# DavidRother/cooking_zoo

Measured on AMD Instinct MI355X. Metric: env-steps/sec at N parallel envs (1/2/4/8 GPU) + achieved HBM GB/s, higher is better.
Workload: dtype u8/u32 state, f64 obs+reward

## Files before the change

### cooking_zoo_amd/csrc/cz_api.hip

```cpp
#include <hip/hip_runtime.h>
#include <dlfcn.h>
#include <stdarg.h>
#include <stdio.h>
#include <stdlib.h>
#include <string.h>

#include <atomic>
#include <string>
#include <vector>

#include "../../include/cookingzoo.h"
#include "cz_launch.h"
#include "cz_generate.h"

using namespace cz;

constexpr int STAT_CHAINS = 256, STAT_COLS = 13;
__global__ __launch_bounds__(64) void k_stats_chains(const uint32_t *__restrict__ su, const double *__restrict__ sf,
                                                     const uint32_t *__restrict__ state, int RW, int N,
                                                     unsigned long long *__restrict__ part ) {
    const int chain = (int)blockIdx.x * 4 + ((int)threadIdx.x >> 4), col = (int)threadIdx.x & 15;
    const int widx = col == 0 ? (int)SU_STEPS : col == 1 ? (int)SU_EPISODES : col == 2 ? (int)SU_LENSUM : col == 3 ? (int)SU_TRUNC
                   : col == 4 ? (int)SU_TERM : col < 9 ? (int)SU_COMPLETED0 + col - 5 : 0;
    const int fidx = (col >= 9 && col < STAT_COLS) ? (int)SF_SUM0 + col - 9 : (int)SF_SUM0;
// ... 264 lines not shown
        double *obs = nullptr, *rew = nullptr; uint8_t *term = nullptr, *trunc = nullptr; hipStream_t stream = nullptr; uint64_t version = 0;
        bool operator==(const RingKey &o) const {
            return ring == o.ring && stride == o.stride && period == o.period && obs == o.obs && rew == o.rew && term == o.term &&
                   trunc == o.trunc && stream == o.stream && version == o.version;
        }
    } ring_key;
    struct RunGraph { int32_t slot, len; hipGraphExec_t ge; uint64_t used; };
    std::vector<RunGraph> ring_graphs;
    uint64_t ring_clock = 0;
    int64_t n_graph_kernels = 0, n_direct_kernels = 0;
    uint64_t tables_version = 0;
    hipEvent_t ev0 = nullptr, ev1 = nullptr;
    bool ktime = false;
    std::vector<hipEvent_t> kev;
    size_t kev_used = 0;
    double ktime_ms = 0.0;
    int64_t klaunches = 0;
    void *rccl = nullptr;
    void *comm = nullptr;
    int n_ranks = 1, rank = 0;
    int wt_override = -1;
    bool lean_enabled = true;
    bool lean_cfg_enabled = true;
    int last_step_variant = -1;
    int last_step_lean = -1;
    int last_step_mode = -1;
    bool huge = false;
    int instance = 0;
    unsigned long long *tl_base = nullptr;
    int32_t tl_cap = 0;
    int64_t tl_count = 0;
    bool graphs_enabled = true;
    bool ring_fused = false;
    int64_t n_ring_fused_steps = 0;
    int32_t graph_min_run = 48;
    int32_t ring_prefix = 0;
    size_t zero_copy_bytes = (size_t)256 << 10;
    cz_stats *d_gather = nullptr;
    std::string err;
};

static thread_local std::string g_err;
static int ready(cz_handle h);
static int set_device(cz_handle h);
static int begin_ranged_call(cz_handle h, int64_t b, int64_t c);
static void mark_ranks(cz_handle h, int32_t first, int32_t count, int ok);
static int flush_updates(cz_handle h, bool force);
// ... 101 lines not shown
    int ndev = 0;
    if (hipGetDeviceCount(&ndev) != hipSuccess || ndev == 0)
        return fail(nullptr, "cz_create: no HIP device available (this library has no CPU fallback)");
    if (cfg->device_id < 0 || cfg->device_id >= ndev) return fail(nullptr, "cz_create: device_id %d out of range", cfg->device_id);
    cz_handle h = new cz_handle_s();
    h->cfg = *cfg;
#define CREATE_CHK(call)                                                                          \
    do {                                                                                          \
        hipError_t _e = (call);                                                                   \
        if (_e != hipSuccess) {                                                                   \
            fail(nullptr, "cz_create: %s failed: %s", #call, hipGetErrorString(_e));             \
            cz_destroy(h);                                                                        \
            return 1;                                                                             \
        }                                                                                         \
    } while (0)
    CREATE_CHK(hipSetDevice(cfg->device_id));
    CREATE_CHK(hipStreamCreateWithFlags(&h->own_stream, hipStreamNonBlocking));
    h->stream = h->own_stream;
    CREATE_CHK(hipEventCreate(&h->ev0));
    CREATE_CHK(hipEventCreate(&h->ev1));
    Params &P = h->P;
    memset(&P, 0, sizeof P);
    P.N = cfg->num_envs; P.A = cfg->num_agents; P.W = cfg->width; P.H = cfg->height; P.D = cfg->max_dyn; P.F = cfg->feat_len;
    const int CW = (C + 3) / 4;
    P.dyn0_off = CELL_WORD0 + CW;
    P.dyn1_off = P.dyn0_off + P.D;
    P.RW = (P.dyn1_off + P.D + 15) / 16 * 16;
    P.scheme = cfg->action_scheme; P.max_steps = cfg->max_steps; P.end_all = cfg->end_condition_all ? 1 : 0;
    P.R = cfg->num_recipes; P.auto_reset = cfg->auto_reset ? 1 : 0; P.env_id_base = cfg->env_id_base;
    P.recipe_reward = cfg->recipe_reward; P.recipe_penalty = cfg->recipe_penalty; P.node_reward = cfg->recipe_node_reward;
    P.time_penalty_step = cfg->max_time_penalty / (double)cfg->max_steps;
    P.T = 1;
    if (const char *s = getenv("CZ_WT")) h->wt_override = atoi(s);
    if (const char *s = getenv("CZ_LEAN")) h->lean_enabled = atoi(s) != 0;
    if (const char *s = getenv("CZ_LEAN_CFG")) h->lean_cfg_enabled = atoi(s) != 0;
    if (const char *s = getenv("CZ_GRAPHS")) h->graphs_enabled = atoi(s) != 0;
    if (const char *s = getenv("CZ_GRAPH_MIN_RUN")) h->graph_min_run = atoi(s) < 4 ? 4 : (atoi(s) > 256 ? 256 : atoi(s));
    if (const char *s = getenv("CZ_RING_PREFIX")) h->ring_prefix = atoi(s) < 0 ? 0 : (atoi(s) > 16 ? 16 : atoi(s));
    if (const char *s = getenv("CZ_ZERO_COPY_BYTES")) h->zero_copy_bytes = (size_t)atoll(s);
#ifdef CZ_SMALL_ONLY
    if (!(P.D <= 64 && C <= 64)) { fail(nullptr, "cz_create: this diagnostic library holds the small kernel instance only"); cz_destroy(h); return 1; }
    h->kl = launchers_small();
#else
    h->instance = (P.D <= 64 && C <= 64) ? 0 : (P.D <= 128 && C <= 256) ? 1 : 2;
    h->kl = h->instance == 0 ? launchers_small() : h->instance == 1 ? launchers_large() : launchers_huge();
#endif
    h->huge = P.D > 128 || C > 256;
    {
        double x = 0.0;
        x += (double)0 * P.node_reward;
        x += 0.0 * P.recipe_reward;
        x += 0.0 * P.recipe_penalty;
        x += P.time_penalty_step;
        P.reward_idle = x;
    }
    const size_t N = (size_t)P.N;
    const size_t state_bytes = N * P.RW * 4;
    CREATE_CHK(hipMalloc(&h->d_state, state_bytes));
// ... 607 lines not shown
};
enum ObsForm { OBS_F64, OBS_CODES, OBS_F32 };

static const char *resolve_step(cz_handle h, const StepCall &c, Params &P, ObsForm &form) {
    uint8_t *const codes = c.fused || c.codes ? c.codes : h->codes;
    float *const obs32 = c.fused || c.obs32 ? c.obs32 : h->obs32;
    if (obs32) {
        if (codes) return "a float32 output (cz_set_f32_output / cz_step_device_f32) and a compact output (cz_set_compact_output / "
                          "cz_step_device_compact) are both set: switch one of them off";
        if (c.obs) return "float32 observation rows are switched on (cz_set_f32_output): pass d_obs = NULL, or switch them off "
                          "with cz_set_f32_output(h, NULL) to get float64 rows";
    }
    form = obs32 ? OBS_F32 : codes ? OBS_CODES : OBS_F64;
    P = h->P;
    P.actions = c.actions; P.obs = c.obs; P.rewards = c.rewards; P.term = c.term; P.trunc = c.trunc; P.marks_out = c.marks;
    P.T = c.T; P.seed = c.seed; P.step0 = c.step0;
    if (obs32) P.obs32 = obs32; else P.codes = codes;
    return nullptr;
}

static hipError_t choose_step(cz_handle h, const Params &P, bool fused, ObsForm form, StepChoice &c) {
    c.lean = false;
    c.cfg = -1;
    if (fused && form == OBS_F32) c.mode = P.actions ? ROLLOUT_ACTIONS_F32 : ROLLOUT_F32;
    else if (fused) c.mode = P.actions ? ROLLOUT_ACTIONS : form != OBS_CODES ? ROLLOUT : P.obs ? ROLLOUT_CODES : ROLLOUT_CODES_ONLY;
    else c.mode = form == OBS_F32 ? STEP_F32 : form == OBS_CODES ? STEP_CODES : STEP;
    if (c.mode == STEP)
        c.lean = h->lean_enabled && h->kl.has_lean && P.obs && !P.marks_out && !P.wide && !(P.auto_reset & 2) && P.F <= 128 * OBS_PAIRS && P.wt == 1;
    if (c.lean && h->lean_cfg_enabled) c.cfg = lean_cfg_of(P);
    return !fused && !P.actions ? hipErrorInvalidValue : hipSuccess;
}

static int launch_step(cz_handle h, const StepCall &call) {
    if ((h->P.auto_reset & 2) && h->spawn_layouts != h->n_layouts)
        return fail(h, "despawn / respawn is on, but the layout pool was reloaded since cz_set_spawn (now %d layouts): call cz_set_spawn "
                       "again (it maps every layout to the level whose spawn areas it uses)", h->n_layouts);
    const hipStream_t stream = h->stream;
    const bool fused = call.fused;
    Params P;
    ObsForm form;
    if (const char *refused = resolve_step(h, call, P, form)) return fail(h, "%s", refused);
    const bool f32 = form == OBS_F32;
    const size_t obs_bytes = (size_t)P.N * P.A * P.F * (f32 ? 4 : 8);
    if (!fused) P.wt = obs_bytes > ((size_t)224 << 20) ? 2 : P.N <= 10240 ? 1 : 0;
    else P.wt = (obs_bytes > ((size_t)224 << 20) && (size_t)P.F * (f32 ? 4 : 8) >= 4096) ? 2 : 0;
    if (h->wt_override >= 0) P.wt = h->wt_override;
    if (!fused) {
        if (!P.rewards) P.rewards = (double *)h->d_dump;
        if (!P.term) P.term = (uint8_t *)h->d_dump;
        if (!P.trunc) P.trunc = (uint8_t *)h->d_dump;
    }
#ifdef CZ_TIMELINE
    P.timeline = (h->tl_base && h->tl_cap > 0) ? h->tl_base + (size_t)(h->tl_count++ % h->tl_cap) * (size_t)P.N * 2 : nullptr;
#endif
    hipEvent_t e0 = nullptr, e1 = nullptr;
    if (h->ktime && caller_capturing(h)) return fail(h, "kernel timing (cz_kernel_time_reset) cannot run inside a stream capture of the caller");
    if (h->ktime) {
        while (h->kev.size() < h->kev_used + 2) {
            hipEvent_t e;
            HIPCHK(h, hipEventCreate(&e));
            h->kev.push_back(e);
        }
        e0 = h->kev[h->kev_used]; e1 = h->kev[h->kev_used + 1];
        h->kev_used += 2;
        HIPCHK(h, hipEventRecord(e0, stream));
    }
    StepChoice choice;
    const hipError_t chosen = choose_step(h, P, fused, form, choice);
    h->last_step_lean = choice.lean ? 1 : 0;
    h->last_step_mode = choice.mode;
    h->last_step_variant = !choice.lean ? -1 : choice.cfg < 0 ? 0 : (0x100 | P.R | (P.end_all << 4) | (P.walk_touches << 5));
    HIPCHK(h, chosen);
    HIPCHK(h, h->kl.step(P, stream, choice));
    if (h->ktime) HIPCHK(h, hipEventRecord(e1, stream));
    return 0;
}
extern "C" int cz_reset(cz_handle h, int64_t b, int64_t c, const int32_t *layout_ids, const uint8_t *recipe_ids,
                        const uint32_t *pool_words, double *obs) {
    if (ready(h) || check_range(h, b, c)) return 1;
    if (c == 0) return 0;
    if (!layout_ids || !recipe_ids) return fail(h, "cz_reset: null argument");
    HIPCHK(h, hipSetDevice(h->cfg.device_id));
    std::vector<uint32_t> pools((size_t)c, 0u);
    for (int64_t i = 0; i < c; ++i) {
        if (layout_ids[i] < 0 || layout_ids[i] >= h->n_layouts) return fail(h, "cz_reset: layout id %d out of range", layout_ids[i]);
        for (int r = 0; r < h->P.R; ++r)
            if (recipe_ids[i * 4 + r] >= h->n_recipes) return fail(h, "cz_reset: recipe id %d out of range", recipe_ids[i * 4 + r]);
        if (pool_words) {
            uint32_t base = pool_words[i] & 0xFFFFu, count = pool_words[i] >> 16;
            if (count && (int)(base + count) > h->n_layouts) return fail(h, "cz_reset: layout pool slice [%u,%u) out of range", base, base + count);
            pools[(size_t)i] = pool_words[i];
        }
    }
    int32_t *const d_lay = h->d_reset_words;
// ... 356 lines not shown
extern "C" int64_t cz_partner_bad_recipes(cz_handle h) {
    if (!h || !h->d_partner) return h ? 0 : -1;
    return read_counter<unsigned long long>(h, partner_counter(h), "cz_partner_bad_recipes");
}
extern "C" int32_t cz_num_actions(cz_handle h) { return h ? (h->P.scheme == 3 ? 5 : 8) : -1; }
extern "C" int cz_action_effects_device(cz_handle h, int64_t b, int64_t c, uint32_t agents, uint32_t ignore, uint8_t *d_mask, uint8_t *d_effects) {
    if (begin_ranged_call(h, b, c)) return 1;
    if (agents == 0 || agents >> h->P.A) return fail(h, "cz_action_effects_device: agents is 0x%x, not a non-empty set of the %d agents", agents, h->P.A);
    if (ignore & ~FX_ALL) return fail(h, "cz_action_effects_device: unknown ignore bits 0x%x", ignore & ~FX_ALL);
    if (!d_mask && !d_effects) return fail(h, "cz_action_effects_device: both output pointers are null");
    if (c == 0) return 0;
    if (set_device(h)) return 1;
    HIPCHK(h, h->kl.action_effects(h->P, h->stream, (int)c, EffectsArgs{b, agents, ignore, d_mask, d_effects}));
    return 0;
}
extern "C" int cz_obs_table_f32(cz_handle h, float *table) {
    if (!h || !table) return fail(h, "cz_obs_table_f32: null argument");
    for (int i = 0; i < LUT_SIZE; ++i) table[i] = (float)h->obs_table[i];
    return 0;
}
extern "C" int32_t cz_diag_last_step_lean(cz_handle h) { return h ? h->last_step_lean : -1; }
extern "C" int32_t cz_diag_last_step_mode(cz_handle h) { return h ? h->last_step_mode : -1; }
extern "C" int32_t cz_diag_last_step_variant(cz_handle h) { return h ? h->last_step_variant : -1; }
extern "C" int32_t cz_diag_instance(cz_handle h) { return h ? h->instance : -1; }
extern "C" int cz_diag_read_layout_pool(cz_handle h, int32_t first, int32_t count, uint32_t *records, uint32_t *desc) {
    if (ready(h)) return 1;
    if (!h->d_lay_init || !h->d_lay_desc) return fail(h, "cz_diag_read_layout_pool: no layout pool loaded");
    if (first < 0 || count < 0 || (int64_t)first + count > h->n_layouts)
        return fail(h, "cz_diag_read_layout_pool: slots [%d, %d) outside the resident pool of %d layouts", first, first + count, h->n_layouts);
    if (count == 0) return 0;
    if (set_device(h)) return 1;
    HIPCHK(h, hipStreamSynchronize(h->stream));
    if (records)
        HIPCHK(h, hipMemcpy(records, h->d_lay_init + (size_t)first * h->P.RW, (size_t)count * h->P.RW * 4, hipMemcpyDeviceToHost));
    if (desc)
        HIPCHK(h, hipMemcpy(desc, h->d_lay_desc + (size_t)first * h->P.F, (size_t)count * h->P.F * 4, hipMemcpyDeviceToHost));
    return 0;
}
extern "C" int cz_obs_table(cz_handle h, double *table) {
    if (!h || !table) return fail(h, "cz_obs_table: null argument");
    memcpy(table, h->obs_table, sizeof h->obs_table);
    return 0;
}
extern "C" const void *cz_obs_table_device(cz_handle h) { return h ? (const void *)h->d_lut : nullptr; }

static bool ring_fusable(cz_handle h, const StepCall &c, int32_t K, int64_t stride);
// ... 593 lines not shown
```

### cooking_zoo_amd/csrc/cz_device.h

```cpp
#pragma once
#include <hip/hip_runtime.h>
#include <stdint.h>
#include <type_traits>

namespace cz {

constexpr int MAX_AGENTS = 4;
constexpr int MAX_NODES = 8;
constexpr int WIDE_NODES = 16;
constexpr int HDR_WORDS = 8;
constexpr int AGENT_WORD0 = HDR_WORDS;
constexpr int RET_WORD0 = HDR_WORDS + MAX_AGENTS;
constexpr int CELL_WORD0 = RET_WORD0 + 2 * MAX_AGENTS;

enum : uint32_t { FLOOR = 0, COUNTER, DELIVERSQUARE, SWITCH, BLOCK, CUTBOARD, BLENDER };
enum : uint32_t { PLATE = 0, ONION, TOMATO, LETTUCE, CARROT, CUCUMBER, BANANA, APPLE, WATERMELON, BREAD };
enum : uint32_t { CELL_TYPE = 7, CELL_READY = 8, CELL_TOGGLE = 16, CELL_ACTIVE = 32, CELL_WALK = 64 };
enum : uint32_t { D_ALIVE = 1u << 24, D_CHOPPED = 2u << 24, D_MASHED = 4u << 24, D_FREE = 8u << 24, D_DONE = 6u << 24 };
enum : uint32_t { COND_NONE = 0, COND_CHOPPED, COND_MASHED, COND_NOT_CHOPPED, COND_NOT_MASHED };
enum : uint32_t { W_T = 0, W_MARKS, W_LAYOUT, W_STATUS, W_EPISODE, W_RECIPES, W_POOL, W_MARKS_HI };
enum : uint32_t { ST_DONE = 1, ST_TERM = 2, ST_TRUNC = 4 };
constexpr int LUT_Y0 = 63, LUT_ZERO = 126, LUT_ONE = 127;
constexpr int LUT_NDONE0 = 128, LUT_CH0 = 132, LUT_MA0 = 136, LUT_CF0 = 140, LUT_OR0 = 144;
enum : uint32_t { SU_EPISODES = 0, SU_STEPS, SU_LENSUM, SU_TRUNC, SU_TERM, SU_COMPLETED0, SU_LAST_LENGTH = 9, SU_LAST_EPISODE, SU_LAST_FLAGS,
// ... 69 lines not shown
static_assert(LEADING_SCALAR_BYTES + sizeof(LeanParams) <= 4 * 64, "the lean argument block: four 64-byte lines with the leading scalars");
#endif
static_assert(LEADING_SCALAR_BYTES + offsetof(LeanParams, obs) + sizeof(double *) == 2 * 64, "the common path's fields end the second line");
struct LeanView : LeanParams {
    uint32_t *state;
    const int32_t *actions;
    const double *lut;
    int32_t N, RW, W, H, D, dyn0_off, dyn1_off;
    static constexpr int32_t wide = 0, wt = 1, T = 1;
    static constexpr uint32_t step0 = 0u;
    static constexpr uint64_t seed = 0u;
    static constexpr uint8_t *codes = nullptr;
    int32_t R, end_all, walk_touches;
    LeanView() = default;
    __host__ __device__ explicit LeanView(const LeanParams &b)
        : LeanParams(b), R((int32_t)(b.settings & 0xFFu)), end_all((int32_t)((b.settings >> 8) & 1u)), walk_touches((int32_t)((b.settings >> 16) & 1u)) {}
};
template <int R_, int END_ALL, int WALK_TOUCHES>
struct LeanViewFixed : LeanView {
    static_assert(R_ >= 1 && R_ <= 4 && (END_ALL | 1) == 1 && (WALK_TOUCHES | 1) == 1, "no such handle");
    static constexpr int32_t R = R_, end_all = END_ALL, walk_touches = WALK_TOUCHES;
    using LeanView::LeanView;
};
template <class PB> using block_of = std::conditional_t<std::is_base_of<LeanParams, PB>::value, LeanParams, Params>;

#ifndef CZ_PRIO
#define CZ_PRIO 1
#endif
#if CZ_PRIO
#define CZ_SETPRIO(p) __builtin_amdgcn_s_setprio(p)
#else
#define CZ_SETPRIO(p) do { } while (0)
#endif
__device__ __forceinline__ uint32_t rfl(uint32_t v) { return __builtin_amdgcn_readfirstlane(v); }
__device__ __forceinline__ uint32_t rdl(uint32_t v, int l) { return __builtin_amdgcn_readlane(v, l); }
__device__ __forceinline__ uint64_t ballot(bool p) { return __builtin_amdgcn_ballot_w64(p); }
__device__ __forceinline__ bool lanes(uint64_t m) { return __builtin_amdgcn_inverse_ballot_w64(m); }
extern "C" __device__ uint32_t __cz_writelane(uint32_t, uint32_t, uint32_t) __asm("llvm.amdgcn.writelane.i32");
__device__ __forceinline__ uint32_t wrl(uint32_t value, int lane, uint32_t into) { return __cz_writelane(value, (uint32_t)lane, into); }

__host__ __device__ inline uint32_t action_hash(uint64_t seed, int64_t env_global, int agent, uint32_t step, uint32_t n) {
    uint32_t x = (uint32_t)seed ^ ((uint32_t)(seed >> 32) * 0x9E3779B1u);
    x ^= (uint32_t)env_global * 0x85EBCA6Bu + (uint32_t)((uint64_t)env_global >> 32) * 0x27D4EB2Fu;
    x ^= ((uint32_t)agent + 1u) * 0xC2B2AE35u;
    x ^= (step + 1u) * 0x165667B1u;
    x ^= x >> 16; x *= 0x7FEB352Du; x ^= x >> 15; x *= 0x846CA68Bu; x ^= x >> 16;
// ... 859 lines not shown
```

### cooking_zoo_amd/csrc/cz_kernels.h

```cpp
#pragma once
#include "cz_device.h"
#include <type_traits>

namespace cz {

#ifdef CZ_PROFILE
#define CZ_STAMP(i)                                                                                    \
    do {                                                                                               \
        unsigned long long _t;                                                                         \
        __builtin_amdgcn_sched_barrier(0);                                                             \
        asm volatile("s_memrealtime %0\n\ts_waitcnt lgkmcnt(0)" : "=s"(_t)::"memory");                 \
        __builtin_amdgcn_sched_barrier(0);                                                             \
        if (lane == 0 && P.stamps) P.stamps[(size_t)env * 16 + (i)] = _t;                               \
    } while (0)
#elif defined(CZ_MARKERS)
#define CZ_STAMP(i) asm volatile("; CZ_MARK " #i)
#else
#define CZ_STAMP(i) do { } while (0)
#endif

typedef const __attribute__((address_space(4))) Params *KParams;
struct StepArgsMirror { uint32_t *a; const int32_t *b; const double *c; int32_t i[8]; Params p; };
struct LeanArgsMirror { uint32_t *a; const int32_t *b; const double *c; int32_t i[8]; LeanParams p; };
static_assert(offsetof(LeanArgsMirror, p) == LEADING_SCALAR_BYTES && offsetof(StepArgsMirror, p) == LEADING_SCALAR_BYTES, "leading scalars");
// ... 22 lines not shown
};
template <int MODE, bool LEAN = false>
struct StepTraits {
    static_assert(MODE >= STEP && MODE <= ROLLOUT_ACTIONS_F32 && (!LEAN || MODE == STEP), "no such variant");
    static constexpr bool fused = MODE == ROLLOUT || MODE == ROLLOUT_ACTIONS || MODE == ROLLOUT_CODES || MODE == ROLLOUT_CODES_ONLY ||
                                  MODE == ROLLOUT_F32 || MODE == ROLLOUT_ACTIONS_F32;
    static constexpr bool ext_actions = MODE == ROLLOUT_ACTIONS || MODE == ROLLOUT_ACTIONS_F32;
    static constexpr bool codes = MODE == STEP_CODES || MODE == ROLLOUT_CODES || MODE == ROLLOUT_CODES_ONLY;
    static constexpr bool codes_only = MODE == ROLLOUT_CODES_ONLY;
    static constexpr bool f32 = MODE == STEP_F32 || MODE == ROLLOUT_F32 || MODE == ROLLOUT_ACTIONS_F32;
    static constexpr bool f64 = !codes_only && !f32;
#ifndef CZ_ROLLOUT_F32_HOLD
#define CZ_ROLLOUT_F32_HOLD 1
#endif
    static constexpr bool desc_held = (codes || f32) && (!fused || codes_only || (f32 && CZ_ROLLOUT_F32_HOLD != 0));
    static constexpr bool desc_per_step = (codes || f32) && fused && !desc_held;
    static constexpr bool lean = LEAN;
    using Block = std::conditional_t<LEAN, LeanParams, Params>;
    using View = std::conditional_t<LEAN, LeanView, Params>;
};
template <int R, int END_ALL, int WALK_TOUCHES>
struct LeanCfgTraits : StepTraits<STEP, true> {
    using View = LeanViewFixed<R, END_ALL, WALK_TOUCHES>;
};

template <int CPL>
struct Img {
    static constexpr bool HUGE = CPL > 4;
    static constexpr int OBJ0 = 0, CELL0 = HUGE ? 1536 : 768, AG0 = CELL0 + (HUGE ? 4096 : 1024), ZERO = AG0 + 32, HALFWORDS = ZERO + 8;
};
constexpr int LUT_ABSENT = 255, LUT_SIZE = 256;
#ifndef CZ_ENVS_PER_WG
#define CZ_ENVS_PER_WG 8
#endif
constexpr int ENVS_PER_WG = CZ_ENVS_PER_WG;
template <int CPL> constexpr int envs_per_wg() { return CPL > 4 ? 4 : ENVS_PER_WG; }
constexpr int OBS_PAIRS = 3;
constexpr int OBS_CHUNK = 2 * OBS_PAIRS;

template <int CPL>
struct Lds {
    int32_t sub[MAX_AGENTS][16];
    uint16_t img[Img<CPL>::HALFWORDS];
    uint64_t locs[CPL <= 4 ? 64 * CPL + 8 : WIDE_NODES * CPL];
};

// ... 134 lines not shown
template <int CPL>
__device__ __forceinline__ void init_lds(const Ctx &cx, Lds<CPL> &s, const CoordWords<CPL> &cw) {
    const int lane = cx.lane;
    s.img[Img<CPL>::ZERO] = (uint16_t)(LUT_ABSENT * 8);
    uint32_t *img32 = reinterpret_cast<uint32_t *>(s.img);
#pragma unroll
    for (int k = 0; k < CPL; ++k) {
        const uint32_t c = (uint32_t)(lane + 64 * k);
        img32[(Img<CPL>::CELL0 >> 1) + 2 * c] = cw.w[k];
    }
}
template <int CPL, class PB>
__device__ __forceinline__ void init_lds(const PB &P, const Ctx &cx, Lds<CPL> &s) {
    const int lane = cx.lane;
    s.img[Img<CPL>::ZERO] = (uint16_t)(LUT_ABSENT * 8);
    uint32_t *img32 = reinterpret_cast<uint32_t *>(s.img);
#pragma unroll
    for (int k = 0; k < CPL; ++k) {
        const uint32_t c = (uint32_t)(lane + 64 * k);
        img32[(Img<CPL>::CELL0 >> 1) + 2 * c] = ldg<uint32_t>(P.lut, COORD_TABLE_OFFSET + c * 4u);
    }
}

template <class PB>
__device__ __forceinline__ void load_desc(const PB &P, uint32_t layout, int chunk, int lane, uint32_t (&dsc)[OBS_CHUNK]) {
    const auto rs = __builtin_amdgcn_make_buffer_rsrc(const_cast<uint32_t *>(P.lay_desc), 0, P.L * P.F * 4, 0x00020000);
    const uint32_t row = layout * (uint32_t)P.F * 4u;
#pragma unroll
    for (int i = 0; i < OBS_CHUNK / 2; ++i) {
        const uint32_t f = (uint32_t)(chunk * (OBS_CHUNK / 2) + i) * 128u + 2u * (uint32_t)lane;
        const uint2_t d = __builtin_bit_cast(uint2_t, __builtin_amdgcn_raw_buffer_load_b64(rs, f * 4u, row, 0));
        dsc[2 * i] = d.x; dsc[2 * i + 1] = d.y;
    }
}

__host__ __device__ inline int codes_pitch(int F) { return (F + 15) & ~15; }
constexpr int CODES_PREFETCH = 2;
struct CodesPrefetch { uint4_t d[CODES_PREFETCH]; uint32_t layout; };
template <class PB>
__device__ __forceinline__ uint4_t load_desc4(const PB &P, uint32_t layout, uint32_t f) {
    const auto rd = __builtin_amdgcn_make_buffer_rsrc(const_cast<uint32_t *>(P.lay_desc), 0, P.L * P.F * 4, 0x00020000);
    return __builtin_bit_cast(uint4_t, __builtin_amdgcn_raw_buffer_load_b128(rd, f * 4u, layout * (uint32_t)P.F * 4u, 0));
}
typedef unsigned short ushort2_t __attribute__((ext_vector_type(2)));
__device__ __forceinline__ uint32_t pk_sub_u16(uint32_t a, uint32_t b) {
    return __builtin_bit_cast(uint32_t, (ushort2_t)(__builtin_bit_cast(ushort2_t, a) - __builtin_bit_cast(ushort2_t, b)));
}
template <int OPL, int CPL, int NA, class PB>
__device__ __forceinline__ void build_image(const PB &P, const Env<OPL, CPL, NA> &e, const Ctx &cx, Lds<CPL> &s, uint32_t submask,
                                            bool objs_changed, bool cells_changed) {
    uint32_t *img32 = reinterpret_cast<uint32_t *>(s.img);
    const uint32_t dead = (uint32_t)(LUT_ABSENT * 8) * 0x10001u;
    const uint32_t c01 = (uint32_t)((P.W - 1) * 8) | ((uint32_t)((LUT_Y0 + P.H - 1) * 8) << 16);
    constexpr uint32_t PICK_XY = 0x0C010C00u;
    if (objs_changed)
#pragma unroll
// ... 101 lines not shown
            int sb[NA][4];
#pragma unroll
            for (int a = 0; a < NA; ++a)
#pragma unroll
                for (int k = 0; k < 4; ++k) sb[a][k] = *reinterpret_cast<const int32_t *>(subb + 64 * a + (dw[k] >> 16));
            const uint32_t p01 = b[0] | (b[1] << 16), p23 = b[2] | (b[3] << 16);
            const int left = P.F - (int)f;
            const uint32_t pad = left >= 4 ? 0u : left <= 0 ? 0xFFFFFFFFu : (0xFFFFFFFFu << (8u * (uint32_t)left));
#pragma unroll
            for (int a = 0; a < NA; ++a) {
                const uint32_t s01 = (uint32_t)sb[a][0] | ((uint32_t)sb[a][1] << 16), s23 = (uint32_t)sb[a][2] | ((uint32_t)sb[a][3] << 16);
                const uint32_t c01 = pk_sub_u16(p01, s01) >> 3, c23 = pk_sub_u16(p23, s23) >> 3;
                __builtin_amdgcn_raw_buffer_store_b32(__builtin_amdgcn_perm(c23, c01, 0x06040200u) | pad, rc[a], f, 0, 16);
            }
        }
    }
    if (!F64 || (!LEAN && !out)) { __builtin_amdgcn_wave_barrier(); return; }
    decltype(__builtin_amdgcn_make_buffer_rsrc(out, 0, 0, 0)) rs[NA];
#pragma unroll
    for (int a = 0; a < NA; ++a) rs[a] = __builtin_amdgcn_make_buffer_rsrc(out + (size_t)a * (uint32_t)P.F, 0, P.F * 8, 0x00020000);
    const uint32_t wt = LEAN ? 1u : (uint32_t)P.wt;
    for (int chunk = 0; LEAN ? chunk == 0 : chunk * 128 * OBS_PAIRS < P.F; ++chunk) {
        if (chunk > 0) load_desc(P, e.layout, chunk, cx.lane, dsc);
        uint32_t b[OBS_CHUNK];
        int sb[NA][OBS_CHUNK];
        double2_t v[NA][OBS_PAIRS];
#pragma unroll
        for (int j = 0; j < OBS_CHUNK; ++j) b[j] = *reinterpret_cast<const uint16_t *>(imgb + (dsc[j] & 0xFFFFu));
#pragma unroll
        for (int a = 0; a < NA; ++a)
#pragma unroll
            for (int j = 0; j < OBS_CHUNK; ++j) sb[a][j] = *reinterpret_cast<const int32_t *>(subb + 64 * a + (dsc[j] >> 16));
#pragma unroll
        for (int a = 0; a < NA; ++a)
#pragma unroll
            for (int i = 0; i < OBS_PAIRS; ++i) {
                v[a][i].x = *reinterpret_cast<const double *>(lutb + ((int)b[2 * i] - sb[a][2 * i]));
                v[a][i].y = *reinterpret_cast<const double *>(lutb + ((int)b[2 * i + 1] - sb[a][2 * i + 1]));
            }
        const uint32_t f0b = (uint32_t)(chunk * OBS_PAIRS * 128 + 2 * cx.lane) * 8u;
#define CZ_OBS_WRITE_ROWS(AUX)                                                                                               \
    _Pragma("unroll") for (int i = 0; i < OBS_PAIRS; ++i)                                                                    \
        _Pragma("unroll") for (int a = 0; a < NA; ++a)                                                                       \
            __builtin_amdgcn_raw_buffer_store_b128(__builtin_bit_cast(uint4_t, v[a][i]), rs[a], f0b + (uint32_t)i * 1024u, 0, AUX)
        if (wt == 1u) { CZ_OBS_WRITE_ROWS(16); }
        else if (wt == 2u) { CZ_OBS_WRITE_ROWS(2); }
        else { CZ_OBS_WRITE_ROWS(0); }
#undef CZ_OBS_WRITE_ROWS
    }
    if (!LEAN && P.F > 128 * OBS_PAIRS) load_desc(P, e.layout, 0, cx.lane, dsc);
    __builtin_amdgcn_wave_barrier();
}

struct StepOut {
    double myrew;
    uint32_t term, trunc;
    bool stepped, finished;
    bool header;
    uint32_t gone;
#ifdef CZ_TIMELINE
    uint32_t dbg;
#endif
};

#define CZ_RARE(hint, x) ((hint) ? __builtin_expect(!!(x), 0) : !!(x))
template <int OPL, int CPL, int NA, int SCHEME, bool FUSED, bool LEAN, class PB>
__device__ __forceinline__ void step_env(const PB &P, unsigned kp_off, Env<OPL, CPL, NA> &e, const Ctx &cx, uint32_t acts,
// ... 161 lines not shown
        o.finished = true;
        o.header = true;
    }
}

struct Early {
    uint32_t *state;
    const int32_t *actions;
    const double *lut;
    int32_t N, RW, W, H, D, dyn0_off, dyn1_off;
};
__host__ __device__ inline Early early_of(const Params &P) {
    return Early{P.state, P.actions, P.lut, P.N, P.RW, P.W, P.H, P.D, P.dyn0_off, P.dyn1_off};
}

template <int OPL, int CPL, int NA, int SCHEME, class V>
__device__ __forceinline__ void step_kernel(uint32_t *e_state, const int32_t *e_actions, const double *e_lut, int32_t e_N,
                                            int32_t e_RW, int32_t e_W, int32_t e_H, int32_t e_D, int32_t e_dyn0,
                                            int32_t e_dyn1, const typename V::Block &P0) {
#ifdef CZ_TIMELINE
    const uint64_t tl_in = wall_clock64();
#endif
    typename V::View P{P0};
    P.state = e_state; P.actions = e_actions; P.lut = e_lut; P.N = e_N; P.RW = e_RW; P.W = e_W; P.H = e_H; P.D = e_D;
    P.dyn0_off = e_dyn0; P.dyn1_off = e_dyn1;
    constexpr int EPW = envs_per_wg<CPL>();
    __shared__ Lds<CPL> lds_all[EPW];
    __shared__ double lut[LUT_SIZE];
    int lane = (int)(threadIdx.x & 63u);
    const int wave = (int)rfl(threadIdx.x >> 6);
    const int env_raw = (int)blockIdx.x * EPW + wave;
    const int env = min(env_raw, P.N - 1);
    static_assert(64 * EPW >= LUT_SIZE, "one table entry per thread");
    const double lutv = ldg<double>(P.lut, min(threadIdx.x, (unsigned)LUT_SIZE - 1u) * 8u);
    constexpr bool SUBMASK_EARLY = CPL == 1;
    uint32_t submask = 0;
    if (SUBMASK_EARLY) submask = load_submask(P, (int)(threadIdx.x & 63u));
    constexpr bool TABLES_EARLY = CPL == 1;
    CoordWords<CPL> coordw{};
    uint32_t rowsel = 0;
    if (TABLES_EARLY) {
        coordw = load_coord_words<CPL>(P, lane);
        rowsel = load_row_selector(P, lane);
    }
    Lds<CPL> &lds = lds_all[wave];
    Ctx cx{P.W, P.H, P.D, P.W * P.H, lane};
    CZ_STAMP(0);
    uint32_t *rec = P.state + (uint32_t)env * (uint32_t)P.RW;
    double *retp = reinterpret_cast<double *>(rec + RET_WORD0);
    int av = 0;
#ifdef CZ_TIMELINE
    const uint64_t tl_seen = wall_clock64();
#endif
    if (!V::fused) av = ldg<int>(P.actions, ((uint32_t)env * (uint32_t)NA + (uint32_t)min(lane, NA - 1)) * 4u);
    double ret = ldg<double>(retp, ((uint32_t)lane & 3u) * 8u);
    Env<OPL, CPL, NA> e;
    load_env<OPL, CPL, NA, V::lean>(P, e, cx, rec);
    if constexpr (TABLES_EARLY) init_lds<CPL>(cx, lds, coordw); else init_lds<CPL>(P, cx, lds);
    uint32_t rowv = TABLES_EARLY ? load_recipe_rows(P, e.recipes, rowsel) : load_recipe_rows(P, e.recipes, lane);
    uint32_t dsc[OBS_CHUNK];
    if (V::f64 && (V::lean || P.obs)) load_desc(P, e.layout, 0, lane, dsc);
    if (!SUBMASK_EARLY) submask = load_submask(P, lane);
    const int64_t env_global = P.env_id_base + env;
    bool cells_dirty = false, objs_dirty = false, header_dirty = V::fused;
    bool img_objs = true, img_cells = true;
    float *const lutf = reinterpret_cast<float *>(lut);
    if (V::f32) { if (threadIdx.x < (unsigned)LUT_SIZE) lutf[threadIdx.x] = (float)lutv; }
    else if (threadIdx.x < (unsigned)LUT_SIZE) lut[threadIdx.x] = lutv;
    __syncthreads();
    if (env_raw >= P.N) return;
    CZ_STAMP(1);
    CodesPrefetch cpre;
    cpre.layout = e.layout;
    if (V::desc_held) {
#pragma unroll
        for (int r = 0; r < CODES_PREFETCH; ++r) cpre.d[r] = load_desc4(P, e.layout, 256u * r + 4u * (uint32_t)lane);
    }

    const int T = V::fused ? P.T : 1;
#ifdef CZ_TIMELINE
    uint32_t tl_dbg = 0u;
#endif
    const uint32_t act_lane = ((uint32_t)env * (uint32_t)NA + (uint32_t)min(lane, NA - 1)) * 4u;
    if (V::ext_actions) av = ldg<int>(e_actions, act_lane);
// ... 128 lines not shown
#define CZ_STEP_ATTR __attribute__((amdgpu_waves_per_eu((!StepTraits<FUSED>::fused && OPL <= 2) ? CZ_STEP_MIN_WPE : 1)))
#else
#define CZ_STEP_ATTR
#endif
template <int OPL, int CPL, int NA, int SCHEME, int FUSED >
__global__ __launch_bounds__(64 * envs_per_wg<CPL>()) CZ_STEP_ATTR void k_step(uint32_t *e_state, const int32_t *e_actions, const double *e_lut, int32_t e_N,
                                                          int32_t e_RW, int32_t e_W, int32_t e_H, int32_t e_D, int32_t e_dyn0,
                                                          int32_t e_dyn1, const Params P0) {
    step_kernel<OPL, CPL, NA, SCHEME, StepTraits<FUSED>>(e_state, e_actions, e_lut, e_N, e_RW, e_W, e_H, e_D, e_dyn0, e_dyn1, P0);
}
template <int OPL, int CPL, int NA, int SCHEME>
__global__ __launch_bounds__(64 * envs_per_wg<CPL>()) void k_step_lean(uint32_t *e_state, const int32_t *e_actions, const double *e_lut, int32_t e_N,
                                                                       int32_t e_RW, int32_t e_W, int32_t e_H, int32_t e_D, int32_t e_dyn0,
                                                                       int32_t e_dyn1, const LeanParams P0) {
    step_kernel<OPL, CPL, NA, SCHEME, StepTraits<STEP, true>>(e_state, e_actions, e_lut, e_N, e_RW, e_W, e_H, e_D, e_dyn0, e_dyn1, P0);
}
template <int OPL, int CPL, int NA, int SCHEME, int R, int END_ALL, int WALK_TOUCHES>
__global__ __launch_bounds__(64 * envs_per_wg<CPL>()) void k_step_lean_cfg(uint32_t *e_state, const int32_t *e_actions, const double *e_lut, int32_t e_N,
                                                                           int32_t e_RW, int32_t e_W, int32_t e_H, int32_t e_D, int32_t e_dyn0,
                                                                           int32_t e_dyn1, const LeanParams P0) {
    step_kernel<OPL, CPL, NA, SCHEME, LeanCfgTraits<R, END_ALL, WALK_TOUCHES>>(e_state, e_actions, e_lut, e_N, e_RW, e_W, e_H, e_D, e_dyn0, e_dyn1, P0);
}

struct StepChoice { StepMode mode; bool lean; int cfg; };
#define CZ_LEAN_CFGS(X) \
    X(1, 3, 1, 0, 0) X(1, 3, 1, 1, 0) X(2, 3, 2, 0, 0) X(2, 3, 2, 1, 0) X(2, 3, 3, 0, 0) X(2, 3, 3, 1, 0) X(2, 3, 4, 0, 0) X(2, 3, 4, 1, 0) \
    X(3, 3, 3, 0, 1)
struct LeanCfg { int A, scheme, R, end_all, walk_touches; };
constexpr LeanCfg LEAN_CFGS[] = {
#define CZ_X(a, s, r, ea, wt) {a, s, r, ea, wt},
    CZ_LEAN_CFGS(CZ_X)
#undef CZ_X
};
constexpr int N_LEAN_CFGS = (int)(sizeof LEAN_CFGS / sizeof LEAN_CFGS[0]);
static_assert(N_LEAN_CFGS <= 16, "build time: each row is one more kernel of the small instance");
inline int lean_cfg_of(const Params &P) {
    for (int i = 0; i < N_LEAN_CFGS; ++i) {
        const LeanCfg &c = LEAN_CFGS[i];
        if (P.A == c.A && P.scheme == c.scheme && P.R == c.R && P.end_all == c.end_all && P.walk_touches == c.walk_touches) return i;
    }
    return -1;
}
inline LeanParams lean_block_of(const Params &P) {
    LeanParams B{};
    B.recipes = P.recipes; B.lay_desc = P.lay_desc; B.L = P.L; B.F = P.F; B.max_steps = P.max_steps; B.auto_reset = P.auto_reset;
    B.reward_idle = P.reward_idle; B.rewards = P.rewards; B.term = P.term; B.trunc = P.trunc; B.obs = P.obs;
    B.settings = (uint32_t)P.R | ((uint32_t)(P.end_all != 0) << 8) | ((uint32_t)(P.walk_touches != 0) << 16);
    B.stat_u = P.stat_u; B.stat_f = P.stat_f; B.lay_init = P.lay_init; B.env_id_base = P.env_id_base;
    B.node_reward = P.node_reward; B.recipe_reward = P.recipe_reward; B.recipe_penalty = P.recipe_penalty; B.time_penalty_step = P.time_penalty_step;
#ifdef CZ_PROFILE
    B.stamps = P.stamps;
#endif
#ifdef CZ_TIMELINE
    B.timeline = P.timeline;
#endif
    return B;
}

template <class F>
inline hipError_t with_agents(int A, F &&f) {
    switch (A) {
    case 1: return f(std::integral_constant<int, 1>{});
// ... 22 lines not shown
```

### cooking_zoo_amd/csrc/cz_launch.h

```cpp
#pragma once
#include "cz_kernels.h"
#include "cz_offstep.h"
#include "cz_query.h"

namespace cz {

struct Launchers {
    hipError_t (*step)(const Params &, hipStream_t, StepChoice);
    hipError_t (*reset)(const Params &, hipStream_t, int64_t, int, const int32_t *, const uint32_t *, const uint32_t *, double *);
    hipError_t (*observe)(const Params &, hipStream_t, int64_t, int, double *, uint8_t *);
    bool has_lean;
    hipError_t (*observe_f32)(const Params &, hipStream_t, int64_t, int, float *);
    hipError_t (*reset_where)(const Params &, hipStream_t, const uint8_t *, const int32_t *, double *, float *, uint8_t *, unsigned long long *);
    hipError_t (*restore_where)(const Params &, hipStream_t, const int32_t *, const uint32_t *, int64_t, uint32_t, double *, float *, uint8_t *,
                                unsigned long long *);
    hipError_t (*set_tasks)(const Params &, hipStream_t, const uint8_t *, const uint32_t *, const uint32_t *, uint32_t, uint64_t, uint32_t,
                            unsigned long long *);
    hipError_t (*observe_grid)(const Params &, hipStream_t, int64_t, int, int32_t, uint32_t *, uint8_t *, float *, int32_t *);
    hipError_t (*navigate)(const Params &, hipStream_t, int64_t, int, int32_t, uint32_t, const int32_t *, int32_t *, int32_t *, uint16_t *);
    hipError_t (*partner)(const Params &, hipStream_t, int, const PartnerArgs &);
    hipError_t (*action_effects)(const Params &, hipStream_t, int, const EffectsArgs &);
    hipError_t (*render)(const Params &, hipStream_t, int, const RenderArgs &);
};

template <int OPL, int CPL, bool HAS_LEAN = false>
struct Inst {
    static hipError_t step(const Params &P, hipStream_t st, StepChoice c) {
        if constexpr (HAS_LEAN) {
            if (c.lean && c.cfg >= 0) {
                if (c.cfg != lean_cfg_of(P)) return hipErrorInvalidValue;
                const LeanParams B = lean_block_of(P);
                int row = 0;
#define CZ_X(a, s, r, ea, wt) if (c.cfg == row++) return launch_step_kernel<CPL>(k_step_lean_cfg<OPL, CPL, a, s, r, ea, wt>, P, B, st);
                CZ_LEAN_CFGS(CZ_X)
#undef CZ_X
                return hipErrorInvalidValue;
            }
        }
        return with_agents(P.A, [&](auto na) {
            return with_scheme(P.scheme, [&](auto scheme) {
                constexpr int NA = decltype(na)::value, S = decltype(scheme)::value;
                if (c.lean) {
                    if constexpr (HAS_LEAN) return launch_step_kernel<CPL>(k_step_lean<OPL, CPL, NA, S>, P, lean_block_of(P), st);
                    return hipErrorInvalidValue;
                }
                switch (c.mode) {
                case STEP: return launch_step_kernel<CPL>(k_step<OPL, CPL, NA, S, STEP>, P, st);
                case ROLLOUT: return launch_step_kernel<CPL>(k_step<OPL, CPL, NA, S, ROLLOUT>, P, st);
                case ROLLOUT_ACTIONS: return launch_step_kernel<CPL>(k_step<OPL, CPL, NA, S, ROLLOUT_ACTIONS>, P, st);
                case STEP_CODES: return launch_step_kernel<CPL>(k_step<OPL, CPL, NA, S, STEP_CODES>, P, st);
                case ROLLOUT_CODES: return launch_step_kernel<CPL>(k_step<OPL, CPL, NA, S, ROLLOUT_CODES>, P, st);
                case ROLLOUT_CODES_ONLY: return launch_step_kernel<CPL>(k_step<OPL, CPL, NA, S, ROLLOUT_CODES_ONLY>, P, st);
                case STEP_F32: return launch_step_kernel<CPL>(k_step<OPL, CPL, NA, S, STEP_F32>, P, st);
                case ROLLOUT_F32: return launch_step_kernel<CPL>(k_step<OPL, CPL, NA, S, ROLLOUT_F32>, P, st);
                case ROLLOUT_ACTIONS_F32: return launch_step_kernel<CPL>(k_step<OPL, CPL, NA, S, ROLLOUT_ACTIONS_F32>, P, st);
// ... 72 lines not shown
```

Measured before the change: 755.8 million.

## Add geometry-specialized lean step kernel with compile-time grid, slots and feature length

Adds a lean step kernel variant whose width, height, slot count, feature length and record offsets are compile-time constants for one specific configuration (7x7 grid, 12 slots, 278 features, 2 agents). With the feature length fixed, the observation write loads and stores only the needed descriptor pairs plus a single 64-bit tail, instead of padding to the full chunk. This removes the runtime loads and address arithmetic for those parameters. The cost is an extra kernel instantiation that only matches one exact geometry, with fallback to the generic lean kernel otherwise.

```diff
diff --git a/cooking_zoo_amd/csrc/cz_api.hip b/cooking_zoo_amd/csrc/cz_api.hip
--- a/cooking_zoo_amd/csrc/cz_api.hip
+++ b/cooking_zoo_amd/csrc/cz_api.hip
@@ -310,7 +310,9 @@
     int wt_override = -1;
     bool lean_enabled = true;
     bool lean_cfg_enabled = true;
+    bool lean_geo_enabled = true;
     int last_step_variant = -1;
+    int last_step_geo = -1;
     int last_step_lean = -1;
     int last_step_mode = -1;
     bool huge = false;
@@ -458,10 +460,8 @@
     Params &P = h->P;
     memset(&P, 0, sizeof P);
     P.N = cfg->num_envs; P.A = cfg->num_agents; P.W = cfg->width; P.H = cfg->height; P.D = cfg->max_dyn; P.F = cfg->feat_len;
-    const int CW = (C + 3) / 4;
-    P.dyn0_off = CELL_WORD0 + CW;
-    P.dyn1_off = P.dyn0_off + P.D;
-    P.RW = (P.dyn1_off + P.D + 15) / 16 * 16;
+    const RecordLayout rl = record_layout(P.W, P.H, P.D);
+    P.dyn0_off = rl.dyn0_off; P.dyn1_off = rl.dyn1_off; P.RW = rl.RW;
     P.scheme = cfg->action_scheme; P.max_steps = cfg->max_steps; P.end_all = cfg->end_condition_all ? 1 : 0;
     P.R = cfg->num_recipes; P.auto_reset = cfg->auto_reset ? 1 : 0; P.env_id_base = cfg->env_id_base;
     P.recipe_reward = cfg->recipe_reward; P.recipe_penalty = cfg->recipe_penalty; P.node_reward = cfg->recipe_node_reward;
@@ -470,6 +470,7 @@
     if (const char *s = getenv("CZ_WT")) h->wt_override = atoi(s);
     if (const char *s = getenv("CZ_LEAN")) h->lean_enabled = atoi(s) != 0;
     if (const char *s = getenv("CZ_LEAN_CFG")) h->lean_cfg_enabled = atoi(s) != 0;
+    if (const char *s = getenv("CZ_LEAN_GEO")) h->lean_geo_enabled = atoi(s) != 0;
     if (const char *s = getenv("CZ_GRAPHS")) h->graphs_enabled = atoi(s) != 0;
     if (const char *s = getenv("CZ_GRAPH_MIN_RUN")) h->graph_min_run = atoi(s) < 4 ? 4 : (atoi(s) > 256 ? 256 : atoi(s));
     if (const char *s = getenv("CZ_RING_PREFIX")) h->ring_prefix = atoi(s) < 0 ? 0 : (atoi(s) > 16 ? 16 : atoi(s));
@@ -1123,12 +1124,14 @@
 static hipError_t choose_step(cz_handle h, const Params &P, bool fused, ObsForm form, StepChoice &c) {
     c.lean = false;
     c.cfg = -1;
+    c.geo = -1;
     if (fused && form == OBS_F32) c.mode = P.actions ? ROLLOUT_ACTIONS_F32 : ROLLOUT_F32;
     else if (fused) c.mode = P.actions ? ROLLOUT_ACTIONS : form != OBS_CODES ? ROLLOUT : P.obs ? ROLLOUT_CODES : ROLLOUT_CODES_ONLY;
     else c.mode = form == OBS_F32 ? STEP_F32 : form == OBS_CODES ? STEP_CODES : STEP;
     if (c.mode == STEP)
         c.lean = h->lean_enabled && h->kl.has_lean && P.obs && !P.marks_out && !P.wide && !(P.auto_reset & 2) && P.F <= 128 * OBS_PAIRS && P.wt == 1;
     if (c.lean && h->lean_cfg_enabled) c.cfg = lean_cfg_of(P);
+    if (c.cfg >= 0 && h->lean_geo_enabled) c.geo = lean_geo_of(P);
     return !fused && !P.actions ? hipErrorInvalidValue : hipSuccess;
 }
 
@@ -1171,6 +1174,7 @@
     h->last_step_lean = choice.lean ? 1 : 0;
     h->last_step_mode = choice.mode;
     h->last_step_variant = !choice.lean ? -1 : choice.cfg < 0 ? 0 : (0x100 | P.R | (P.end_all << 4) | (P.walk_touches << 5));
+    h->last_step_geo = choice.geo;
     HIPCHK(h, chosen);
     HIPCHK(h, h->kl.step(P, stream, choice));
     if (h->ktime) HIPCHK(h, hipEventRecord(e1, stream));
@@ -1573,6 +1577,23 @@
 extern "C" int32_t cz_diag_last_step_lean(cz_handle h) { return h ? h->last_step_lean : -1; }
 extern "C" int32_t cz_diag_last_step_mode(cz_handle h) { return h ? h->last_step_mode : -1; }
 extern "C" int32_t cz_diag_last_step_variant(cz_handle h) { return h ? h->last_step_variant : -1; }
+extern "C" int32_t cz_diag_last_step_geo(cz_handle h) { return h ? h->last_step_geo : -1; }
+extern "C" int32_t cz_diag_lean_geo_row(int32_t row, int32_t *out) {
+    if (!out) return N_LEAN_GEOS;
+    if (row < 0 || row >= N_LEAN_GEOS) return -1;
+    int32_t v[12];
+    int i = 0;
+#define CZ_X(a, s, r, ea, wt, w, h, d, f)                                                                                          \
+    if (row == i++) {                                                                                                              \
+        using V = LeanViewGeo<r, ea, wt, w, h, d, f>;                                                                              \
+        const int32_t q[12] = {a, s, V::R, V::end_all, V::walk_touches, V::W, V::H, V::D, V::F, V::RW, V::dyn0_off, V::dyn1_off};   \
+        memcpy(v, q, sizeof v);                                                                                                    \
+    }
+    CZ_LEAN_GEOS(CZ_X)
+#undef CZ_X
+    memcpy(out, v, sizeof v);
+    return N_LEAN_GEOS;
+}
 extern "C" int32_t cz_diag_instance(cz_handle h) { return h ? h->instance : -1; }
 extern "C" int cz_diag_read_layout_pool(cz_handle h, int32_t first, int32_t count, uint32_t *records, uint32_t *desc) {
     if (ready(h)) return 1;
diff --git a/cooking_zoo_amd/csrc/cz_device.h b/cooking_zoo_amd/csrc/cz_device.h
--- a/cooking_zoo_amd/csrc/cz_device.h
+++ b/cooking_zoo_amd/csrc/cz_device.h
@@ -115,6 +115,27 @@
     static constexpr int32_t R = R_, end_all = END_ALL, walk_touches = WALK_TOUCHES;
     using LeanView::LeanView;
 };
+struct RecordLayout { int32_t dyn0_off, dyn1_off, RW; };
+__host__ __device__ constexpr RecordLayout record_layout(int W, int H, int D) {
+    const int dyn0 = HDR_WORDS + MAX_AGENTS + 2 * MAX_AGENTS + (W * H + 3) / 4;
+    return RecordLayout{dyn0, dyn0 + D, (dyn0 + 2 * D + 15) / 16 * 16};
+}
+template <int R_, int END_ALL, int WALK_TOUCHES, int W_, int H_, int D_, int F_>
+struct LeanViewGeo : LeanViewFixed<R_, END_ALL, WALK_TOUCHES> {
+    static_assert(W_ >= 1 && H_ >= 1 && W_ * H_ <= 64 && D_ >= 1 && D_ <= 64 && F_ >= 1 && F_ <= 384, "the small instance: one cell and one slot per lane, one chunk of features");
+    static constexpr int32_t W = W_, H = H_, D = D_, F = F_;
+    static constexpr int32_t dyn0_off = record_layout(W_, H_, D_).dyn0_off, dyn1_off = record_layout(W_, H_, D_).dyn1_off, RW = record_layout(W_, H_, D_).RW;
+    using LeanViewFixed<R_, END_ALL, WALK_TOUCHES>::LeanViewFixed;
+};
+template <class PB> struct FixedRowLength { static constexpr int value = 0; };
+template <int R_, int END_ALL, int WALK_TOUCHES, int W_, int H_, int D_, int F_>
+struct FixedRowLength<LeanViewGeo<R_, END_ALL, WALK_TOUCHES, W_, H_, D_, F_>> { static constexpr int value = F_; };
+template <class PB>
+__device__ __forceinline__ void take_leading_scalars(PB &P, uint32_t *state, const int32_t *actions, const double *lut, int32_t N, int32_t RW,
+                                                     int32_t W, int32_t H, int32_t D, int32_t dyn0, int32_t dyn1) {
+    P.state = state; P.actions = actions; P.lut = lut; P.N = N;
+    if constexpr (FixedRowLength<PB>::value == 0) { P.RW = RW; P.W = W; P.H = H; P.D = D; P.dyn0_off = dyn0; P.dyn1_off = dyn1; }
+}
 template <class PB> using block_of = std::conditional_t<std::is_base_of<LeanParams, PB>::value, LeanParams, Params>;
 
 #ifndef CZ_PRIO
diff --git a/cooking_zoo_amd/csrc/cz_kernels.h b/cooking_zoo_amd/csrc/cz_kernels.h
--- a/cooking_zoo_amd/csrc/cz_kernels.h
+++ b/cooking_zoo_amd/csrc/cz_kernels.h
@@ -68,6 +68,10 @@
 template <int R, int END_ALL, int WALK_TOUCHES>
 struct LeanCfgTraits : StepTraits<STEP, true> {
     using View = LeanViewFixed<R, END_ALL, WALK_TOUCHES>;
+};
+template <int R, int END_ALL, int WALK_TOUCHES, int W, int H, int D, int F>
+struct LeanGeoTraits : StepTraits<STEP, true> {
+    using View = LeanViewGeo<R, END_ALL, WALK_TOUCHES, W, H, D, F>;
 };
 
 template <int CPL>
@@ -248,16 +252,29 @@
     }
 }
 
+#ifndef CZ_GEO_TAIL
+#define CZ_GEO_TAIL 1
+#endif
+template <int F>
+struct ObsSplit {
+    static constexpr int full = F / 128 < OBS_PAIRS ? F / 128 : OBS_PAIRS, rest = F - 128 * full;
+    static constexpr bool tail = CZ_GEO_TAIL != 0 && F > 0 && rest >= 1 && rest <= 64;
+    static constexpr int pairs = F == 0 ? OBS_PAIRS : tail ? full : (F + 127) / 128;
+    static_assert(F <= 128 * OBS_PAIRS && 2 * pairs + (tail ? 1 : 0) <= OBS_CHUNK, "one chunk");
+};
 template <class PB>
 __device__ __forceinline__ void load_desc(const PB &P, uint32_t layout, int chunk, int lane, uint32_t (&dsc)[OBS_CHUNK]) {
+    using Split = ObsSplit<FixedRowLength<PB>::value>;
     const auto rs = __builtin_amdgcn_make_buffer_rsrc(const_cast<uint32_t *>(P.lay_desc), 0, P.L * P.F * 4, 0x00020000);
     const uint32_t row = layout * (uint32_t)P.F * 4u;
 #pragma unroll
-    for (int i = 0; i < OBS_CHUNK / 2; ++i) {
+    for (int i = 0; i < Split::pairs; ++i) {
         const uint32_t f = (uint32_t)(chunk * (OBS_CHUNK / 2) + i) * 128u + 2u * (uint32_t)lane;
         const uint2_t d = __builtin_bit_cast(uint2_t, __builtin_amdgcn_raw_buffer_load_b64(rs, f * 4u, row, 0));
         dsc[2 * i] = d.x; dsc[2 * i + 1] = d.y;
     }
+    if constexpr (Split::tail)
+        dsc[2 * Split::pairs] = (uint32_t)__builtin_amdgcn_raw_buffer_load_b32(rs, (128u * Split::pairs + (uint32_t)lane) * 4u, row, 0);
 }
 
 __host__ __device__ inline int codes_pitch(int F) { return (F + 15) & ~15; }
@@ -405,27 +422,36 @@
     const uint32_t wt = LEAN ? 1u : (uint32_t)P.wt;
     for (int chunk = 0; LEAN ? chunk == 0 : chunk * 128 * OBS_PAIRS < P.F; ++chunk) {
         if (chunk > 0) load_desc(P, e.layout, chunk, cx.lane, dsc);
+        using Split = ObsSplit<FixedRowLength<PB>::value>;
+        constexpr int PAIRS = Split::pairs, WORDS = 2 * PAIRS + (Split::tail ? 1 : 0);
         uint32_t b[OBS_CHUNK];
         int sb[NA][OBS_CHUNK];
         double2_t v[NA][OBS_PAIRS];
-#pragma unroll
-        for (int j = 0; j < OBS_CHUNK; ++j) b[j] = *reinterpret_cast<const uint16_t *>(imgb + (dsc[j] & 0xFFFFu));
+        [[maybe_unused]] double vt[NA];
+#pragma unroll
+        for (int j = 0; j < WORDS; ++j) b[j] = *reinterpret_cast<const uint16_t *>(imgb + (dsc[j] & 0xFFFFu));
 #pragma unroll
         for (int a = 0; a < NA; ++a)
 #pragma unroll
-            for (int j = 0; j < OBS_CHUNK; ++j) sb[a][j] = *reinterpret_cast<const int32_t *>(subb + 64 * a + (dsc[j] >> 16));
-#pragma unroll
-        for (int a = 0; a < NA; ++a)
-#pragma unroll
-            for (int i = 0; i < OBS_PAIRS; ++i) {
+            for (int j = 0; j < WORDS; ++j) sb[a][j] = *reinterpret_cast<const int32_t *>(subb + 64 * a + (dsc[j] >> 16));
+#pragma unroll
+        for (int a = 0; a < NA; ++a) {
+#pragma unroll
+            for (int i = 0; i < PAIRS; ++i) {
                 v[a][i].x = *reinterpret_cast<const double *>(lutb + ((int)b[2 * i] - sb[a][2 * i]));
                 v[a][i].y = *reinterpret_cast<const double *>(lutb + ((int)b[2 * i + 1] - sb[a][2 * i + 1]));
             }
+            if constexpr (Split::tail) vt[a] = *reinterpret_cast<const double *>(lutb + ((int)b[2 * PAIRS] - sb[a][2 * PAIRS]));
+        }
         const uint32_t f0b = (uint32_t)(chunk * OBS_PAIRS * 128 + 2 * cx.lane) * 8u;
 #define CZ_OBS_WRITE_ROWS(AUX)                                                                                               \
-    _Pragma("unroll") for (int i = 0; i < OBS_PAIRS; ++i)                                                                    \
+    _Pragma("unroll") for (int i = 0; i < PAIRS; ++i)                                                                        \
         _Pragma("unroll") for (int a = 0; a < NA; ++a)                                                                       \
-            __builtin_amdgcn_raw_buffer_store_b128(__builtin_bit_cast(uint4_t, v[a][i]), rs[a], f0b + (uint32_t)i * 1024u, 0, AUX)
+            __builtin_amdgcn_raw_buffer_store_b128(__builtin_bit_cast(uint4_t, v[a][i]), rs[a], f0b + (uint32_t)i * 1024u, 0, AUX); \
+    if constexpr (Split::tail) {                                                                                             \
+        _Pragma("unroll") for (int a = 0; a < NA; ++a)                                                                       \
+            __builtin_amdgcn_raw_buffer_store_b64(__builtin_bit_cast(uint2_t, vt[a]), rs[a], (uint32_t)(128 * PAIRS + cx.lane) * 8u, 0, AUX); \
+    }
         if (wt == 1u) { CZ_OBS_WRITE_ROWS(16); }
         else if (wt == 2u) { CZ_OBS_WRITE_ROWS(2); }
         else { CZ_OBS_WRITE_ROWS(0); }
@@ -633,8 +659,7 @@
     const uint64_t tl_in = wall_clock64();
 #endif
     typename V::View P{P0};
-    P.state = e_state; P.actions = e_actions; P.lut = e_lut; P.N = e_N; P.RW = e_RW; P.W = e_W; P.H = e_H; P.D = e_D;
-    P.dyn0_off = e_dyn0; P.dyn1_off = e_dyn1;
+    take_leading_scalars(P, e_state, e_actions, e_lut, e_N, e_RW, e_W, e_H, e_D, e_dyn0, e_dyn1);
     constexpr int EPW = envs_per_wg<CPL>();
     __shared__ Lds<CPL> lds_all[EPW];
     __shared__ double lut[LUT_SIZE];
@@ -671,6 +696,7 @@
     uint32_t rowv = TABLES_EARLY ? load_recipe_rows(P, e.recipes, rowsel) : load_recipe_rows(P, e.recipes, lane);
     uint32_t dsc[OBS_CHUNK];
     if (V::f64 && (V::lean || P.obs)) load_desc(P, e.layout, 0, lane, dsc);
+    if constexpr (FixedRowLength<typename V::View>::value != 0) asm volatile("" ::"s"(P0.F), "s"(P0.max_steps));
     if (!SUBMASK_EARLY) submask = load_submask(P, lane);
     const int64_t env_global = P.env_id_base + env;
     bool cells_dirty = false, objs_dirty = false, header_dirty = V::fused;
@@ -845,7 +871,14 @@
     step_kernel<OPL, CPL, NA, SCHEME, LeanCfgTraits<R, END_ALL, WALK_TOUCHES>>(e_state, e_actions, e_lut, e_N, e_RW, e_W, e_H, e_D, e_dyn0, e_dyn1, P0);
 }
 
-struct StepChoice { StepMode mode; bool lean; int cfg; };
+template <int OPL, int CPL, int NA, int SCHEME, int R, int END_ALL, int WALK_TOUCHES, int W, int H, int D, int F>
+__global__ __launch_bounds__(64 * envs_per_wg<CPL>()) void k_step_lean_geo(uint32_t *e_state, const int32_t *e_actions, const double *e_lut, int32_t e_N,
+                                                                           int32_t e_RW, int32_t e_W, int32_t e_H, int32_t e_D, int32_t e_dyn0,
+                                                                           int32_t e_dyn1, const LeanParams P0) {
+    step_kernel<OPL, CPL, NA, SCHEME, LeanGeoTraits<R, END_ALL, WALK_TOUCHES, W, H, D, F>>(e_state, e_actions, e_lut, e_N, e_RW, e_W, e_H, e_D, e_dyn0, e_dyn1, P0);
+}
+
+struct StepChoice { StepMode mode; bool lean; int cfg; int geo; };
 #define CZ_LEAN_CFGS(X) \
     X(1, 3, 1, 0, 0) X(1, 3, 1, 1, 0) X(2, 3, 2, 0, 0) X(2, 3, 2, 1, 0) X(2, 3, 3, 0, 0) X(2, 3, 3, 1, 0) X(2, 3, 4, 0, 0) X(2, 3, 4, 1, 0) \
     X(3, 3, 3, 0, 1)
@@ -861,6 +894,26 @@
     for (int i = 0; i < N_LEAN_CFGS; ++i) {
         const LeanCfg &c = LEAN_CFGS[i];
         if (P.A == c.A && P.scheme == c.scheme && P.R == c.R && P.end_all == c.end_all && P.walk_touches == c.walk_touches) return i;
+    }
+    return -1;
+}
+#define CZ_LEAN_GEOS(X) \
+    X(2, 3, 2, 0, 0, 7, 7, 12, 278)
+struct LeanGeo { LeanCfg cfg; int W, H, D, F; };
+constexpr LeanGeo LEAN_GEOS[] = {
+#define CZ_X(a, s, r, ea, wt, w, h, d, f) {{a, s, r, ea, wt}, w, h, d, f},
+    CZ_LEAN_GEOS(CZ_X)
+#undef CZ_X
+};
+constexpr int N_LEAN_GEOS = (int)(sizeof LEAN_GEOS / sizeof LEAN_GEOS[0]);
+static_assert(N_LEAN_GEOS <= 4, "build time: each row is one more kernel of the small instance");
+inline int lean_geo_of(const Params &P) {
+    for (int i = 0; i < N_LEAN_GEOS; ++i) {
+        const LeanGeo &g = LEAN_GEOS[i];
+        const RecordLayout rl = record_layout(g.W, g.H, g.D);
+        if (P.A == g.cfg.A && P.scheme == g.cfg.scheme && P.R == g.cfg.R && P.end_all == g.cfg.end_all && P.walk_touches == g.cfg.walk_touches &&
+            P.W == g.W && P.H == g.H && P.D == g.D && P.F == g.F && P.RW == rl.RW && P.dyn0_off == rl.dyn0_off && P.dyn1_off == rl.dyn1_off)
+            return i;
     }
     return -1;
 }
diff --git a/cooking_zoo_amd/csrc/cz_launch.h b/cooking_zoo_amd/csrc/cz_launch.h
--- a/cooking_zoo_amd/csrc/cz_launch.h
+++ b/cooking_zoo_amd/csrc/cz_launch.h
@@ -31,6 +31,13 @@
                 if (c.cfg != lean_cfg_of(P)) return hipErrorInvalidValue;
                 const LeanParams B = lean_block_of(P);
                 int row = 0;
+                if (c.geo >= 0) {
+                    if (c.geo != lean_geo_of(P)) return hipErrorInvalidValue;
+#define CZ_X(a, s, r, ea, wt, w, h, d, f) if (c.geo == row++) return launch_step_kernel<CPL>(k_step_lean_geo<OPL, CPL, a, s, r, ea, wt, w, h, d, f>, P, B, st);
+                    CZ_LEAN_GEOS(CZ_X)
+#undef CZ_X
+                    return hipErrorInvalidValue;
+                }
 #define CZ_X(a, s, r, ea, wt) if (c.cfg == row++) return launch_step_kernel<CPL>(k_step_lean_cfg<OPL, CPL, a, s, r, ea, wt>, P, B, st);
                 CZ_LEAN_CFGS(CZ_X)
 #undef CZ_X
```

Result: slower. 708.4 million (-6.3%).
